# UoB-HPC/neutral

Measured on AMD Instinct MI355X. Metric: particle-steps/sec, higher is better.
Workload: dtype f64

## Files before the change

### neutral_amd/csrc/neutral_tiled.hip

```cpp
#include <cstdlib>
#include <cstring>
#include <type_traits>

#include "neutral_kernels.h"

#include "neutral_device.h"
#include "neutral_history.h"
#include "neutral_wave.h"

namespace neutral {

#ifndef NEUTRAL_STREAM_BLOCK
#define NEUTRAL_STREAM_BLOCK 1024
#endif
constexpr int kStreamBlock = NEUTRAL_STREAM_BLOCK;
constexpr int kChunkParticlesMax = 32768;
constexpr int kChunkParticlesMin = 1024;
constexpr int kStreamRefillMin = 56;
constexpr int kStreamRepeat = 64;
constexpr int kStreamRepeatOnePass = 128;
#ifdef NEUTRAL_NO_CARRIED_START
constexpr bool kCarriedStart = false;
#else
constexpr bool kCarriedStart = true;
// ... 342 lines not shown
                                                                    const unsigned* slot_of_id,
                                                                    ParticleView p, int n,
                                                                    const int* abort_flag,
                                                                    const unsigned* first_inactive,
                                                                    unsigned final_from,
                                                                    const unsigned* skip_ids,
                                                                    int partial_ok) {
  if (abort_flag && *abort_flag) {
    return;
  }
  for (long long kk = (long long)blockIdx.x * kSortBlock + threadIdx.x; kk < n; kk += (long long)gridDim.x * kSortBlock) {
    const int k = (int)kk;
    if (skip_ids && ((skip_ids[k >> 5] >> (k & 31)) & 1u)) {
      continue;
    }
    const unsigned slot = slot_of_id[k];
    if (slot >= (first_inactive ? *first_inactive : final_from)) {
      continue;
    }
    const rec_quad* const q = (const rec_quad*)__builtin_assume_aligned(&rec[slot], 16);
    ParticleRec r;
    rec_quad* const rq = (rec_quad*)&r;
    rq[0] = q[0];
    rq[1] = q[1];
    rq[2] = q[2];
    __builtin_nontemporal_store(r.x, &p.x[k]);
    __builtin_nontemporal_store(r.y, &p.y[k]);
    __builtin_nontemporal_store(r.dt_to_census, &p.dt_to_census[k]);
    __builtin_nontemporal_store(r.mfp_to_collision, &p.mfp_to_collision[k]);
    __builtin_nontemporal_store(r.cellx, &p.cellx[k]);
    __builtin_nontemporal_store(r.celly, &p.celly[k]);
    if (!partial_ok || (r.dead & kRecChanged)) {
      rq[3] = q[3];
      rq[4] = q[4];
      __builtin_nontemporal_store(r.omega_x, &p.omega_x[k]);
      __builtin_nontemporal_store(r.omega_y, &p.omega_y[k]);
      __builtin_nontemporal_store(r.energy, &p.energy[k]);
      __builtin_nontemporal_store(r.weight, &p.weight[k]);
      __builtin_nontemporal_store((record_state(r.dead) == kRecDead) ? 1 : 0, &p.dead[k]);
    }
  }
}

__global__ __launch_bounds__(1024) void tile_chunks_kernel(TiledArgs t) {
  __shared__ unsigned s_chunks[1024];
  constexpr int kStagedOffsets = 8192;
  __shared__ unsigned s_offset[kStagedOffsets + 2];
  const int tid = threadIdx.x;
  const bool staged = t.nsort + 1 <= kStagedOffsets;
  if (staged) {
    for (int i = tid; i <= t.nsort + 1; i += 1024) {
      s_offset[i] = t.tile_offset[i];
    }
    __syncthreads();
  }
  const unsigned* offset = staged ? s_offset : t.tile_offset;
  const unsigned nactive = offset[t.nsort];
  const int classes = t.reach_classes;
  long long per = (t.ntiles + 1023) / 1024;
  if (nactive > 0) {
    const long long per_sparse =
        ((long long)t.chunk_particles * (long long)t.ntiles + nactive - 1) / (long long)nactive;
    per = (per_sparse > per) ? per_sparse : per;
    constexpr long long kSweepTilesMax = 32;
    const long long floor_per = (t.ntiles + 1023) / 1024;
    const long long cap = (floor_per > kSweepTilesMax) ? floor_per : kSweepTilesMax;
    per = (per > cap) ? cap : per;
  }
  per = (per > t.ntiles) ? t.ntiles : per;
  const long long lo_ll = (long long)tid * per;
  const int lo = (lo_ll < t.ntiles) ? (int)lo_ll : t.ntiles;
  const int hi = (lo_ll + per < t.ntiles) ? (int)(lo_ll + per) : t.ntiles;
  const unsigned cp = (unsigned)t.chunk_particles;

  unsigned nch = 0;
  unsigned chunk = 0;
  unsigned nwindowed = 0;
  for (int sweep = 0; sweep < 2; ++sweep) {
    unsigned run_begin = 0, run_end = 0;
    auto emit = [&](unsigned begin, unsigned end, unsigned tile, unsigned windowed) {
      if (end <= begin) {
        return;
      }
      const unsigned parts = (end - begin + cp - 1) / cp;
      const unsigned size = (end - begin + parts - 1) / parts;
      for (unsigned b = begin; b < end; b += size) {
        const unsigned e = (b + size < end) ? b + size : end;
        if (sweep == 0) {
          nch++;
        } else {
          const unsigned w = (windowed && (e - b) >= (unsigned)t.window_min_particles) ? 1u : 0u;
          if (chunk < (unsigned)t.max_chunks) {
            t.chunks[chunk] = make_uint4(b, e, tile, w);
          }
          nwindowed += w;
          chunk++;
        }
      }
    };
    for (int i = lo; i < hi; ++i) {
      const unsigned begin = offset[i * classes];
      const unsigned end = offset[(i + 1) * classes];
      if (end - begin >= (unsigned)t.window_min_particles) {
        emit(run_begin, run_end, 0u, 0u);
        run_begin = run_end = end;
        emit(begin, end, (unsigned)i, 1u);
      } else {
        if (run_end == run_begin) {
          run_begin = begin;
        }
        run_end = end;
      }
    }
    emit(run_begin, run_end, 0u, 0u);
    if (sweep == 0) {
      s_chunks[tid] = nch;
      __syncthreads();
      for (int off = 1; off < 1024; off <<= 1) {
        const unsigned c0 = (tid >= off) ? s_chunks[tid - off] : 0;
        __syncthreads();
        s_chunks[tid] += c0;
        __syncthreads();
      }
      chunk = s_chunks[tid] - nch;
    }
  }
  if (nwindowed) {
    atomicAdd(&t.ctrl[kCtrlWindowed], nwindowed);
  }
  if (tid == 1023) {
    t.ctrl[kCtrlNumChunks] = s_chunks[1023];
    t.ctrl[kCtrlActive] = nactive;
    t.ctrl[kCtrlLive] = nactive;
    t.ctrl[kCtrlChunkHead] = 0;
    t.ctrl[kCtrlCollideCount] = 0;
    t.ctrl[kCtrlMigrants] = 0;
    if (t.pass == 0) {
      t.ctrl[kCtrlPassesUsed] = 1;
      t.ctrl[kCtrlEmigrants] = 0;
      t.ctrl[kCtrlFirstInactive] = offset[t.nsort];
    } else if (nactive > 0) {
      t.ctrl[kCtrlPassesUsed] = (unsigned)t.pass + 1u;
    }
  }
}

__global__ __launch_bounds__(kSortBlock) void tile_uniform_kernel(SolveArgs a, TiledArgs t, int window_cells) {
  __shared__ int s_differs;
  if (threadIdx.x == 0) {
    s_differs = 0;
  }
  __syncthreads();
  const int tile = (int)blockIdx.x;
  const int margin = (window_cells - (1 << t.tile_shift)) >> 1;
  int x0 = ((tile % t.tiles_x) << t.tile_shift) - margin - 1;
  int y0 = ((tile / t.tiles_x) << t.tile_shift) - margin - 1;
  int x1 = x0 + window_cells + 2;
  int y1 = y0 + window_cells + 2;
  x0 = (x0 < 0) ? 0 : x0;
  y0 = (y0 < 0) ? 0 : y0;
  x1 = (x1 > a.nx) ? a.nx : x1;
  y1 = (y1 > a.ny) ? a.ny : y1;
  const int w = x1 - x0;
  const int n = w * (y1 - y0);
  const long long first = __double_as_longlong(a.density[(size_t)y0 * a.nx + x0]);
  bool differs = false;
  for (int i = threadIdx.x; i < n; i += kSortBlock) {
    const int y = y0 + i / w;
    const int x = x0 + i % w;
    differs |= (__double_as_longlong(a.density[(size_t)y * a.nx + x]) != first);
  }
  if (__ballot(differs) != 0 && (threadIdx.x & 63) == 0) {
    s_differs = 1;
  }
  __syncthreads();
  if (threadIdx.x == 0) {
    t.tile_uniform[tile] = s_differs ? 0 : 1;
  }
}

__global__ __launch_bounds__(1024) void edges_check_kernel(SolveArgs a, TiledArgs t) {
  __shared__ int s_differs;
  if (threadIdx.x == 0) {
    s_differs = 0;
  }
  __syncthreads();
  bool differs = !(a.edge_dx > 0.0) || !(a.edge_dy > 0.0);
  for (int i = threadIdx.x; i <= a.nx; i += 1024) {
    differs |= __double_as_longlong(edge_from_formula(a.edge_dx, i + a.x_off)) !=
               __double_as_longlong(a.edgex[i + a.pad]);
  }
  for (int i = threadIdx.x; i <= a.ny; i += 1024) {
    differs |= __double_as_longlong(edge_from_formula(a.edge_dy, i + a.y_off)) !=
               __double_as_longlong(a.edgey[i + a.pad]);
  }
  if (__ballot(differs) != 0 && (threadIdx.x & 63) == 0) {
    s_differs = 1;
  }
  __syncthreads();
  if (threadIdx.x == 0) {
    *t.edges_computed = s_differs ? 0 : 1;
  }
}


__global__ __launch_bounds__(kSortBlock) void queue_reset_kernel(TiledArgs t) {
  const int tile = (int)blockIdx.x;
  unsigned used = t.queue_tail[tile];
  used = (used > t.queue_capacity) ? t.queue_capacity : used;
  unsigned* log = t.queue_entries + (size_t)tile * t.queue_capacity;
  for (unsigned i = threadIdx.x; i < used; i += kSortBlock) {
    log[i] = kQueueEmpty;
  }
  __syncthreads();
  if (threadIdx.x == 0) {
    t.queue_tail[tile] = 0u;
    t.queue_head[tile] = 0u;
  }
}

template <int kW>
__device__ __forceinline__ void flush_window(const SolveArgs& a, double* window, double* mesh,
                                             int ox, int oy) {
  constexpr int kS = kW + kWindowRowPad;
  for (int i = threadIdx.x; i < kW * kW; i += kStreamBlock) {
    const int at = (i / kW) * kS + (i % kW);
    const double v = window[at];
    window[at] = 0.0;
    if (v != 0.0) {
      const int gx = ox + (i % kW);
      const int gy = oy + (i / kW);
      if (gx >= 0 && gx < a.nx && gy >= 0 && gy < a.ny) {
        unsafeAtomicAdd(&mesh[gy * a.nx + gx], v);
      }
    }
  }
}

template <bool kSameTables, bool kWithIndex = true>
__host__ __device__ __forceinline__ size_t stream_lds_payload_bytes(const SolveArgs& a, int window_cells) {
  size_t lds = sizeof(double) * (size_t)window_cells;
  if (kWithIndex && a.scatter_index) {
    lds += sizeof(unsigned short) * (size_t)(a.scatter_index_n + 1);
  }
  if (kWithIndex && !kSameTables && a.absorb_index) {
    lds += sizeof(unsigned short) * (size_t)(a.absorb_index_n + 1);
  }
  return (lds + 15) & ~(size_t)15;
}
#ifdef NEUTRAL_PHASE_CLOCK
constexpr size_t kStreamLdsControlBytes = 64 + 16 * 9 * 8;
#else
constexpr size_t kStreamLdsControlBytes = 64;
#endif

__device__ __forceinline__ bool far_to_go(const History& h, const TiledArgs& t) {
  const double ahead = h.speed * h.dt_to_census;
  const double facets_ahead = ahead * (fabs(h.omega_x) * t.cells_per_x +
                                       fabs(h.omega_y) * t.cells_per_y);
  return facets_ahead > kMigrateMinFacets;
}

#ifdef NEUTRAL_PHASE_CLOCK
__device__ unsigned long long g_phase_clock[8];
#define PHASE_DECL                                                                              \
  unsigned long long* const lds_ph =                                                            \
      (unsigned long long*)((char*)lds_ctl + 64) + (threadIdx.x >> 6) * 9;                      \
  if ((threadIdx.x & 63) == 0) {                                                                \
    lds_ph[0] = __builtin_readcyclecounter();                                                   \
    for (int k = 1; k <= 8; ++k) lds_ph[k] = 0;                                                 \
  }
#define PHASE(k)                                                                                \
  do {                                                                                          \
    if ((int)(threadIdx.x & 63) == __builtin_ctzll(__builtin_amdgcn_ballot_w64(true))) {        \
      const unsigned long long ph_now = __builtin_readcyclecounter();                           \
      lds_ph[1 + (k)] += ph_now - lds_ph[0];                                                    \
      lds_ph[0] = ph_now;                                                                       \
    }                                                                                           \
  } while (0)
#define PHASE_REPORT                                                                            \
  if ((threadIdx.x & 63) == 0) {                                                                \
    for (int k = 0; k < 8; ++k) atomicAdd(&g_phase_clock[k], lds_ph[1 + k]);                    \
  }
extern "C" void neutral_hip_debug_phase_clock(unsigned long long* out8) {
  (void)hipDeviceSynchronize();
  (void)hipMemcpyFromSymbol(out8, HIP_SYMBOL(g_phase_clock), sizeof(unsigned long long) * 8);
  unsigned long long zero[8] = {0, 0, 0, 0, 0, 0, 0, 0};
  (void)hipMemcpyToSymbol(HIP_SYMBOL(g_phase_clock), zero, sizeof(zero));
}
#else
#define PHASE_DECL
#define PHASE(k)
#define PHASE_REPORT
#endif

static __device__ SpectrumParams d_spectrum = {};

static __global__ void spectrum_params_kernel(SpectrumParams p) { d_spectrum = p; }

static __device__ CurrentParams d_current = {nullptr, nullptr, nullptr};

static __global__ void current_params_kernel(CurrentParams p) { d_current = p; }

template <bool kSameTables, bool kFlux, bool kDomain, bool kChecked, bool kQueues, bool kSpectrum = false,
          bool kCurrent = false>
__global__ __launch_bounds__(kStreamBlock) void stream_kernel(SolveArgs a, TiledArgs t) {
  constexpr bool kCarried = kCarriedStart && kSameTables && !kDomain && !kQueues;
  constexpr int kW = WindowTallyT<kFlux, kCarried, false, kCurrent>::W;
  constexpr int kWindows = window_count(kFlux, kCurrent);
  extern __shared__ double lds_raw[];
  constexpr int kWindowDoubles = kW * (kW + kWindowRowPad);
  double* window = lds_raw;
  unsigned short* lds_index = (unsigned short*)(lds_raw + kWindows * kWindowDoubles);
  int* const lds_ctl = (int*)((char*)lds_raw + stream_lds_payload_bytes<kSameTables, !kCarried>(a, kWindows * kWindowDoubles));
  int& s_chunk = lds_ctl[0];
  int& s_end = lds_ctl[1];
  int& s_tile = lds_ctl[2];
  int& s_windowed = lds_ctl[3];
  int& s_cursor = lds_ctl[4];
  int& s_kind = lds_ctl[5];
  unsigned& s_best = ((unsigned*)lds_ctl)[6];
  int& s_best_tile = lds_ctl[7];

  if (a.abort_flag && *a.abort_flag) {
    return;
  }
  clock_stamp_begin(a.counters);
  CsLookup<const unsigned short*> ix{nullptr, nullptr};
  {
    int used = 0;
    if (!kCarried && a.scatter_index) {
      for (int i = threadIdx.x; i <= a.scatter_index_n; i += kStreamBlock) {
        lds_index[i] = a.scatter_index[i];
      }
      ix.scatter_index = lds_index;
      used = a.scatter_index_n + 1;
    }
    if (!kCarried && !kSameTables && a.absorb_index) {
      for (int i = threadIdx.x; i <= a.absorb_index_n; i += kStreamBlock) {
        lds_index[used + i] = a.absorb_index[i];
      }
      ix.absorb_index = lds_index + used;
    }
    for (int i = threadIdx.x; i < kWindows * kWindowDoubles; i += kStreamBlock) {
      window[i] = 0.0;
    }
  }
  WindowTallyT<kFlux, kCarried, kSpectrum, kCurrent> tally{(lds_double*)window, 0, 0, SpectrumView{},
                                                           kCurrent ? &d_current : nullptr};
  if (kSpectrum) {
    tally.spectrum = spectrum_view(&d_spectrum, (lds_double*)((char*)lds_ctl + kStreamLdsControlBytes));
    spectrum_bins_zero(tally.spectrum);
  }

  const int nchunks = (int)t.ctrl[kCtrlNumChunks];
  const bool edges_computed =
      t.edges_computed && __builtin_amdgcn_readfirstlane(*t.edges_computed) != 0;
  const bool budget_on = t.allow_migrate && (kQueues || t.ctrl[kCtrlWindowed] != 0);
  int cur_tile = -1;
  int win_ox = 0;
  int win_oy = 0;

  unsigned nfacets = 0;
  unsigned w_processed = 0;
  unsigned w_census = 0;
  unsigned w_migrants = 0;
  unsigned w_emigrants = 0;

  History h;
  h.ev = kEvEnd;
  spectrum_lane_start(h, tally);
  int pid = -1;

  const bool queues = kQueues && t.allow_migrate;
  const unsigned qcap = t.queue_capacity;
  unsigned w_ended = 0;
  unsigned w_hops = 0;
  unsigned w_overflows = 0;
  unsigned wg_batches = 0;
  unsigned wg_idle_polls = 0;
  enum : int { kWorkChunk = 0, kWorkQueue = 1, kWorkNone = 2 };

  PHASE_DECL
  for (;;) {
    if (queues && (threadIdx.x & 63) == 0 && w_ended) {
      atomicSub(&t.ctrl[kCtrlLive], w_ended);
    }
    w_ended = 0;
    unsigned polls = 0;
    for (;;) {
      __syncthreads();
      auto claim = [&](int tile, unsigned at_least) -> bool {
        for (;;) {
          const unsigned head = __hip_atomic_load(&t.queue_head[tile], __ATOMIC_RELAXED, __HIP_MEMORY_SCOPE_AGENT);
          unsigned tail = __hip_atomic_load(&t.queue_tail[tile], __ATOMIC_RELAXED, __HIP_MEMORY_SCOPE_AGENT);
          tail = (tail > qcap) ? qcap : tail;
          if (tail <= head || tail - head < at_least) {
            return false;
          }
          unsigned m = tail - head;
          m = (m > kQueueBatchMax) ? kQueueBatchMax : m;
          if (atomicCAS(&t.queue_head[tile], head, head + m) == head) {
            s_cursor = (int)head;
            s_end = (int)(head + m);
            s_tile = tile;
            s_windowed = 1;
            return true;
          }
        }
      };
      if (threadIdx.x == 0) {
        s_best = 0u;
        s_best_tile = -1;
        int kind = kWorkNone;
        if (queues && cur_tile >= 0 && claim(cur_tile, kQueueStayMin)) {
          kind = kWorkQueue;
          wg_batches++;
        }
        if (kind == kWorkNone &&
            __hip_atomic_load(&t.ctrl[kCtrlChunkHead], __ATOMIC_RELAXED, __HIP_MEMORY_SCOPE_AGENT) < (unsigned)nchunks) {
          const int c = (int)atomicAdd(&t.ctrl[kCtrlChunkHead], 1u);
          if (c < nchunks) {
            const uint4 ch = t.chunks[c];
            s_cursor = (int)ch.x;
            s_end = (int)ch.y;
            s_tile = (int)ch.z;
            s_windowed = (int)ch.w;
            kind = kWorkChunk;
          }
        }
        s_kind = kind;
      }
      __syncthreads();
      if (__builtin_amdgcn_readfirstlane(s_kind) != kWorkNone) {
        break;
      }
      if (!queues) {
        break;
      }
      {
        const int start = (cur_tile >= 0) ? cur_tile : (int)((blockIdx.x * 2654435761u) % (unsigned)t.ntiles);
        unsigned mine = 0u;
        int mine_tile = -1;
        for (int tile = (int)threadIdx.x; tile < t.ntiles; tile += kStreamBlock) {
          unsigned tail = __hip_atomic_load(&t.queue_tail[tile], __ATOMIC_RELAXED, __HIP_MEMORY_SCOPE_AGENT);
          const unsigned head = __hip_atomic_load(&t.queue_head[tile], __ATOMIC_RELAXED, __HIP_MEMORY_SCOPE_AGENT);
          tail = (tail > qcap) ? qcap : tail;
          if (tail > head) {
            const unsigned waiting = tail - head;
            unsigned key;
            if (waiting >= kQueueBatchMin) {
              int ahead = tile - start;
              ahead += (ahead < 0) ? t.ntiles : 0;
              key = 0x80000000u | (unsigned)(t.ntiles - ahead);
            } else {
              const unsigned salt = ((unsigned)tile * 2654435761u + blockIdx.x * 40503u + polls * 9973u) >> 22;
              key = (waiting << 10) | salt;
            }
            if (key > mine) {
              mine = key;
              mine_tile = tile;
            }
          }
        }
        unsigned most = mine;
#pragma unroll
        for (int off = 32; off > 0; off >>= 1) {
          const unsigned other = __shfl_xor(most, off, 64);
          most = (other > most) ? other : most;
        }
        const unsigned long long m_top = __ballot(most != 0u && mine == most);
        if (m_top != 0ull && __builtin_ctzll(m_top) == (int)(threadIdx.x & 63)) {
          atomicMax(&s_best, most);
        }
        __syncthreads();
        if (mine != 0u && mine == s_best) {
          s_best_tile = mine_tile;
        }
        __syncthreads();
      }
      if (threadIdx.x == 0) {
        int kind = kWorkNone;
        if (s_best != 0u && claim(s_best_tile, 1u)) {
          kind = kWorkQueue;
        }
        s_kind = kind;
        if (kind == kWorkQueue) {
          wg_batches++;
        }
        s_chunk = 0;
        if (kind == kWorkNone) {
          const unsigned live = __hip_atomic_load(&t.ctrl[kCtrlLive], __ATOMIC_RELAXED, __HIP_MEMORY_SCOPE_AGENT);
          if (live == 0u) {
            s_chunk = -1;
          } else if (s_best != 0u) {
          } else if (polls >= kQueueIdlePollsMax) {
            atomicAdd(&a.counters->aborted, 1u);
            s_chunk = -1;
          } else {
            wg_idle_polls++;
            const unsigned nap = (polls < 5u) ? polls : 5u;
            for (unsigned k = 0; k < (1u << nap); ++k) {
              __builtin_amdgcn_s_sleep(64);
            }
          }
        }
      }
      __syncthreads();
      if (__builtin_amdgcn_readfirstlane(s_kind) != kWorkNone || __builtin_amdgcn_readfirstlane(s_chunk) < 0) {
        break;
      }
      polls++;
    }
    const int work = __builtin_amdgcn_readfirstlane(s_kind);
    PHASE(0);
    if (work == kWorkNone) {
      break;
    }
    const bool from_queue = (work == kWorkQueue);
    const bool fresh = !from_queue && t.pass == 0;
    const int chunk_end = __builtin_amdgcn_readfirstlane(s_end);
    const int chunk_tile = __builtin_amdgcn_readfirstlane(s_tile);
    const bool windowed = (__builtin_amdgcn_readfirstlane(s_windowed) != 0);
    if (windowed && chunk_tile != cur_tile) {
      if (cur_tile >= 0) {
        flush_window<kW>(a, window, a.tally, win_ox, win_oy);
        if (kFlux) {
          flush_window<kW>(a, window + kWindowDoubles, a.flux_tally, win_ox, win_oy);
        }
        if (kCurrent) {
          flush_window<kW>(a, window + 2 * kWindowDoubles, d_current.jx, win_ox, win_oy);
          flush_window<kW>(a, window + 3 * kWindowDoubles, d_current.jy, win_ox, win_oy);
        }
      }
      cur_tile = chunk_tile;
      const int margin = (kW - (1 << t.tile_shift)) >> 1;
      win_ox = ((cur_tile % t.tiles_x) << t.tile_shift) - margin;
      win_oy = ((cur_tile / t.tiles_x) << t.tile_shift) - margin;
      __syncthreads();
    }
    PHASE(1);
    const bool uniform_window =
        windowed && t.tile_uniform &&
        __builtin_amdgcn_readfirstlane((int)t.tile_uniform[cur_tile]) != 0;
    double window_density = 0.0;
    if (kCarried && uniform_window) {
      const int tile_x = (cur_tile % t.tiles_x) << t.tile_shift;
      const int tile_y = (cur_tile / t.tiles_x) << t.tile_shift;
      window_density = a.density[(size_t)tile_y * (size_t)a.nx + (size_t)tile_x];
    }
    unsigned long long may_migrate =
        __builtin_amdgcn_readfirstlane((windowed && t.allow_migrate) ? 1 : 0) ? ~0ull : 0ull;
    asm volatile("" : "+s"(may_migrate));
    tally.ox = __builtin_amdgcn_readfirstlane(windowed ? win_ox : (1 << 30));
    tally.oy = __builtin_amdgcn_readfirstlane(windowed ? win_oy : (1 << 30));

    bool has = false;
    bool drained = false;
    for (;;) {
      const unsigned long long m_empty = __ballot(!has);
      const int n_empty = drained ? 0 : __popcll(m_empty);
      const int n_stream = 64 - __popcll(m_empty);
      if (n_empty + n_stream == 0) {
        break;
      }
      int park = kRecIdle;
      bool did_census = false;
      bool ended = false;
      if (n_empty >= t.refill_min || n_stream == 0) {
        int base = 0;
        if ((threadIdx.x & 63) == 0) {
          base = atomicAdd(&s_cursor, n_empty);
        }
        base = __builtin_amdgcn_readfirstlane(base);
        if (base >= chunk_end) {
          drained = true;
        } else {
          const int mine = base + lane_rank(m_empty);
          if (fresh) {
            const int left = chunk_end - base;
            w_processed += (unsigned)((n_empty < left) ? n_empty : left);
          }
          if (!has && mine < chunk_end) {
            unsigned src;
            if (from_queue) {
              const unsigned* place = t.queue_entries + ((size_t)chunk_tile * qcap + (size_t)mine);
              unsigned spins = 0;
              do {
                src = __hip_atomic_load(place, __ATOMIC_RELAXED, __HIP_MEMORY_SCOPE_AGENT);
              } while (src == kQueueEmpty && ++spins < (1u << 22));
            } else {
              src = t.order[mine];
            }
            if (src >= (unsigned)a.nparticles) {
              atomicAdd(&a.counters->aborted, 1u);
              ended = true;
            } else {
            pid = fresh ? mine : (int)src;
            double micro = 0.0, minus_log_rn0 = 0.0;
            if (kCarried) {
              const CarriedStart cs = fresh ? t.carried_in[src] : t.carried_out[src];
              micro = cs.micro;
              minus_log_rn0 = cs.minus_log_rn0;
            }
            bool bad_load = false;
            if (from_queue || (queues && !fresh)) {
              load_record_through(h, a, t.rec_out[src], true);
              if (from_queue) {
                const int want_tile = ((h.celly - a.y_off) >> t.tile_shift) * t.tiles_x + ((h.cellx - a.x_off) >> t.tile_shift);
                bad_load = (want_tile != chunk_tile) | (!kDomain && (h.id & ~kIdChanged) >= (unsigned)a.nparticles);
              }
            } else {
              load_record(h, a, fresh ? t.rec_in[src] : t.rec_out[src], !fresh);
            }
            if (fresh) {
              t.id_out[pid] = h.id;
              if (!kDomain && t.slots_by_id) {
                t.slot_of_id[h.id] = (unsigned)pid;
              }
              if (kCarried) {
                t.carried_out[pid].micro = micro;
              }
            }
            if (bad_load) {
              atomicAdd(&a.counters->aborted, 1u);
              ended = true;
            } else {
            if (kCarried) {
              if (fresh) {
                prologue_carried<kChecked>(h, a, micro, minus_log_rn0, uniform_window, window_density);
              } else {
                resume_carried<kChecked>(h, a, micro, uniform_window, window_density);
              }
            } else if (fresh) {
              prologue<kSameTables, kChecked>(h, a, ix);
            } else {
              resume<kSameTables, kChecked>(h, a, ix);
            }
            if (!kDomain) {
              h.counter = 1;
            }
            h.plain_div = 0;
            refresh_speed_reciprocal<kChecked>(h);
            refresh_mfp_reciprocal<kChecked>(h);
            h.dep_rate = deposit_rate(h, a);
            spectrum_regroup(h, tally);
            if (edges_computed) {
              load_targets<true>(h, a);
            } else {
              load_targets<false>(h, a);
            }
            decide_carried(h);
            h.nevents++;
            has = true;
            if (h.ev == kEvCollision) {
              park = kRecCollide;
            }
            }
            }
          }
        }
        PHASE(2);
      } else if (has) {
        if (h.ev == kEvFacet) {
          int crossed = 0;
          h.m_x_facet = __builtin_amdgcn_ballot_w64(h.x_facet != 0);

          auto run_facets = [&](auto uniform_density, auto computed_edges) {
          constexpr bool kUniform = decltype(uniform_density)::value;
          constexpr bool kEdges = decltype(computed_edges)::value;
          WindowCellTallyT<kFlux, kUniform, kCarried, kSpectrum, kCurrent> cell_tally{
              tally.window, (unsigned)(h.cellx - a.x_off - tally.ox),
              (unsigned)(h.celly - a.y_off - tally.oy), 0ull, tally.spectrum, tally.current_meshes};
          bool out_of_window = cell_tally.outside();
          cell_tally.m_outside = __builtin_amdgcn_ballot_w64(out_of_window);
          bool run = true;
          if ((cell_tally.m_outside & may_migrate) != 0) {
            asm volatile("");
            if (out_of_window) {
              run = !far_to_go(h, t);
            }
          }
          PHASE(3);
          if (run) {
#pragma unroll 1
            do {
              cross_facet<kChecked, true, kDomain ? 1 : 0, true, kEdges>(h, a, cell_tally);
              asm("v_add_u32_e32 %0, 1, %0" : "+v"(crossed));
              if (kDomain) {
                if (outside_domain(h, a)) {
                  park = kRecEmigrate;
                  break;
                }
              }
              cell_tally.lx = (unsigned)(h.cellx - a.x_off - tally.ox);
              cell_tally.ly = (unsigned)(h.celly - a.y_off - tally.oy);
              out_of_window = cell_tally.outside();
              cell_tally.m_outside = __builtin_amdgcn_ballot_w64(out_of_window);
              run = surely_next_is_facet(h) & (crossed < t.stream_repeat);
              if ((cell_tally.m_outside & may_migrate) != 0) {
                asm volatile("");
                if (out_of_window) {
                  run = run & !far_to_go(h, t);
                }
              }
            } while (run);
          }
          PHASE(5);
          };
          if (uniform_window) {
            if (edges_computed) {
              run_facets(std::true_type{}, std::true_type{});
            } else {
              run_facets(std::true_type{}, std::false_type{});
            }
          } else {
            if (edges_computed) {
              run_facets(std::false_type{}, std::true_type{});
            } else {
              run_facets(std::false_type{}, std::false_type{});
            }
          }
          decide_carried(h);
          park = (park == kRecIdle && h.ev == kEvCollision) ? (int)kRecCollide : park;
          if (windowed && t.allow_migrate && park == kRecIdle && h.ev == kEvFacet) {
            const unsigned lx = (unsigned)(h.cellx - a.x_off - tally.ox);
            const unsigned ly = (unsigned)(h.celly - a.y_off - tally.oy);
            if (!((lx < (unsigned)kW) & (ly < (unsigned)kW)) && far_to_go(h, t)) {
              park = kRecMigrate;
            }
          }
          nfacets += (unsigned)crossed;
          h.nevents += (unsigned)crossed;
          if (!windowed && budget_on && park == kRecIdle && h.ev == kEvFacet &&
              h.nevents >= kUnwindowedBudget) {
            const double ahead = h.speed * h.dt_to_census;
            if (ahead * (fabs(h.omega_x) * t.cells_per_x + fabs(h.omega_y) * t.cells_per_y) >
                kMigrateMinFacets) {
              park = kRecMigrate;
            }
          }
          if (h.nevents > kMaxEventsPerHistory && h.ev == kEvFacet && park == kRecIdle) {
            atomicAdd(&a.counters->aborted, 1u);
            h.ev = kEvEnd;
          }
          PHASE(3);
        } else {
          if (h.ev == kEvCensus) {
            census_streamed<kChecked>(h, a, tally);
          }
          store_record(h, a, t.rec_out[pid], kRecIdle);
          t.info_out[pid] = slot_summary(
              kRecIdle, h.cellx - a.x_off, h.celly - a.y_off, t.tiles_x, t.tile_shift,
              t.reach_classes > 1 ? reach_class(h.omega_x, h.omega_y, h.cellx - a.x_off,
                                                h.celly - a.y_off, t.tile_shift, kW, t.cells_per_x,
                                                t.cells_per_y)
                                  : 0u);
          has = false;
          ended = true;
          did_census = (h.ev == kEvCensus);
          PHASE(6);
        }
      }
      bool queued = false;
      const bool hop = queues && park == kRecMigrate;
      const unsigned long long m_hop = __ballot(hop);
      if (m_hop != 0ull) {
        int dest = 0;
        if (hop) {
          dest = ((h.celly - a.y_off) >> t.tile_shift) * t.tiles_x + ((h.cellx - a.x_off) >> t.tile_shift);
          if ((unsigned)dest >= (unsigned)t.ntiles || (unsigned)pid >= (unsigned)a.nparticles) {
            atomicAdd(&a.counters->aborted, 1u);
            dest = 0;
          }
          store_record_through(h, a, t.rec_out[(unsigned)pid < (unsigned)a.nparticles ? pid : 0], kRecMigrate);
        }
        int leader = -1;
        unsigned rank = 0, group = 0;
        unsigned long long todo = m_hop;
        while (todo != 0ull) {
          const int l = __builtin_ctzll(todo);
          const int tile_l = __builtin_amdgcn_readlane(dest, l);
          const unsigned long long same = __ballot(hop && dest == tile_l);
          if (hop && dest == tile_l) {
            leader = l;
            rank = (unsigned)lane_rank(same);
            group = (unsigned)__popcll(same);
          }
          todo &= ~same;
        }
        drain_stores();
        unsigned base = 0;
        if (hop && leader == (int)(threadIdx.x & 63)) {
          base = atomicAdd(&t.queue_tail[dest], group);
        }
        base = (unsigned)__shfl((int)base, leader < 0 ? 0 : leader, 64);
        if (hop) {
          const unsigned place = base + rank;
          if (place < qcap) {
            __hip_atomic_store(t.queue_entries + ((size_t)dest * qcap + (size_t)place), (unsigned)pid,
                               __ATOMIC_RELAXED, __HIP_MEMORY_SCOPE_AGENT);
            queued = true;
            has = false;
          }
        }
        w_hops += (unsigned)__popcll(__ballot(queued));
        w_overflows += (unsigned)__popcll(__ballot(hop && !queued));
      }
      if (park != kRecIdle && !queued) {
        if (!hop) {
          store_record(h, a, t.rec_out[pid], park);
        }
        t.info_out[pid] = slot_summary(
            park, h.cellx - a.x_off, h.celly - a.y_off, t.tiles_x, t.tile_shift,
            (t.reach_classes > 1 && park == kRecMigrate)
                ? reach_class(h.omega_x, h.omega_y, h.cellx - a.x_off, h.celly - a.y_off,
                              t.tile_shift, kW, t.cells_per_x, t.cells_per_y)
                : 0u);
        has = false;
        ended = true;
      }
      PHASE(7);
      w_ended += (unsigned)__popcll(__ballot(ended));
      w_migrants += (unsigned)__popcll(__ballot(park == kRecMigrate && !queued));
      if (kDomain) {
        w_emigrants += (unsigned)__popcll(__ballot(park == kRecEmigrate));
      }
      w_census += (unsigned)__popcll(__ballot(did_census));
    }
  }
  PHASE(0);
  PHASE_REPORT
  if ((threadIdx.x & 63) == 0 && w_migrants) {
    atomicAdd(&t.ctrl[kCtrlMigrants], w_migrants);
  }
  if ((threadIdx.x & 63) == 0 && w_hops) {
    atomicAdd(&t.ctrl[kCtrlHops], w_hops);
  }
  if ((threadIdx.x & 63) == 0 && w_overflows) {
    atomicAdd(&t.ctrl[kCtrlOverflows], w_overflows);
  }
  if (threadIdx.x == 0 && wg_batches) {
    atomicAdd(&t.ctrl[kCtrlBatches], wg_batches);
  }
  if (threadIdx.x == 0 && wg_idle_polls) {
    atomicAdd(&t.ctrl[kCtrlIdlePolls], wg_idle_polls);
  }
  if (kDomain && (threadIdx.x & 63) == 0 && w_emigrants) {
    atomicAdd(&t.ctrl[kCtrlEmigrants], w_emigrants);
  }
  if (cur_tile >= 0) {
    flush_window<kW>(a, window, a.tally, win_ox, win_oy);
    if (kFlux) {
      flush_window<kW>(a, window + kWindowDoubles, a.flux_tally, win_ox, win_oy);
    }
    if (kCurrent) {
      flush_window<kW>(a, window + 2 * kWindowDoubles, d_current.jx, win_ox, win_oy);
      flush_window<kW>(a, window + 3 * kWindowDoubles, d_current.jy, win_ox, win_oy);
    }
  }
  spectrum_finish(h, tally, d_spectrum.buffer, a.inv_ntotal_particles);
  {
    const unsigned wf = wave_sum_u32(nfacets);
    if ((threadIdx.x & 63) == 0) {
      if (w_processed) atomicAdd(&a.counters->nprocessed, (unsigned long long)w_processed);
      if (wf) atomicAdd(&a.counters->nfacets, (unsigned long long)wf);
      if (w_census) atomicAdd(&a.counters->ncensus, (unsigned long long)w_census);
    }
  }
  clock_stamp_end(a.counters);
}


__device__ __forceinline__ int owner_rank(const DomainGrid& d, int cellx, int celly) {
  int rx = cellx / d.bx;
  int ry = celly / d.by;
  rx = (rx < 0) ? 0 : ((rx >= d.px) ? d.px - 1 : rx);
  ry = (ry < 0) ? 0 : ((ry >= d.py) ? d.py - 1 : ry);
  return ry * d.px + rx;
}

__global__ __launch_bounds__(kSortBlock) void emigrant_count_kernel(const ParticleRec* rec,
                                                                    const unsigned* info, int n,
                                                                    DomainGrid d, unsigned* counts) {
  const int i = blockIdx.x * kSortBlock + threadIdx.x;
  if (i < n && summary_state(info[i]) == kRecEmigrate) {
    atomicAdd(&counts[owner_rank(d, rec[i].cellx, rec[i].celly)], 1u);
  }
}

__global__ __launch_bounds__(kSortBlock) void emigrant_pack_kernel(ParticleRec* rec, unsigned* info,
                                                                   int n, DomainGrid d,
                                                                   const unsigned* offset,
                                                                   unsigned* cursor,
                                                                   ParticleRec* send, int tiles_x,
                                                                   int tile_shift,
                                                                   unsigned* free_slots,
                                                                   unsigned* nfree) {
  const int i = blockIdx.x * kSortBlock + threadIdx.x;
  if (i < n && summary_state(info[i]) == kRecEmigrate) {
    ParticleRec r = rec[i];
    const int dest = owner_rank(d, r.cellx, r.celly);
    const unsigned k = atomicAdd(&cursor[dest], 1u);
    free_slots[atomicAdd(nfree, 1u)] = (unsigned)i;
    const unsigned counter = record_counter(r.dead);
    r.dead = record_word(kRecMigrate, counter);
    send[offset[dest] + k] = r;
    rec[i].dead = record_word(kRecGone, 0u);
    info[i] = slot_summary(kRecGone, 0, 0, tiles_x, tile_shift);
  }
}

__global__ __launch_bounds__(kSortBlock) void immigrant_append_kernel(const ParticleRec* recv,
                                                                      int nrecv, ParticleRec* rec,
                                                                      unsigned* info, unsigned* ids,
                                                                      int first_slot, int x_off,
                                                                      int y_off, int tiles_x,
                                                                      int tile_shift,
                                                                      unsigned* migrants,
                                                                      const unsigned* free_slots,
                                                                      int nfree, int reuse) {
  const int j = blockIdx.x * kSortBlock + threadIdx.x;
  if (j == 0) {
    atomicAdd(migrants, (unsigned)nrecv);
  }
  if (j < nrecv) {
    const ParticleRec r = recv[j];
    const int slot = (j < reuse) ? (int)free_slots[nfree - 1 - j] : first_slot + (j - reuse);
    rec[slot] = r;
    ids[slot] = r.id;
    info[slot] = slot_summary(kRecMigrate, r.cellx - x_off, r.celly - y_off, tiles_x, tile_shift);
  }
}

__global__ __launch_bounds__(kSortBlock) void compact_records_kernel(
    const ParticleRec* rec, const unsigned* info, const unsigned* ids, int n, ParticleRec* rec_to,
    unsigned* info_to, unsigned* ids_to, unsigned* cursor) {
  const int i = blockIdx.x * kSortBlock + threadIdx.x;
  const bool keep = i < n && summary_state(info[i]) != kRecGone;
  const unsigned long long m = __ballot(keep);
  unsigned base = 0;
  if ((threadIdx.x & 63) == 0 && m) {
    base = atomicAdd(cursor, (unsigned)__popcll(m));
  }
  base = __builtin_amdgcn_readfirstlane(base);
  if (keep) {
    const unsigned j = base + (unsigned)lane_rank(m);
    rec_to[j] = rec[i];
    info_to[j] = info[i];
    ids_to[j] = ids[i];
  }
}

__global__ __launch_bounds__(kSortBlock) void import_by_slot_kernel(ParticleView p,
                                                                    const unsigned* keys,
                                                                    ParticleRec* rec, unsigned* info,
                                                                    unsigned* ids, int tiles_x,
                                                                    int tile_shift, int x_off,
                                                                    int y_off, int n) {
  const int i = blockIdx.x * kSortBlock + threadIdx.x;
  if (i < n) {
    ParticleRec r;
    r.x = p.x[i];
    r.y = p.y[i];
    r.omega_x = p.omega_x[i];
    r.omega_y = p.omega_y[i];
    r.energy = p.energy[i];
    r.weight = p.weight[i];
    r.dt_to_census = p.dt_to_census[i];
    r.mfp_to_collision = p.mfp_to_collision[i];
    r.cellx = p.cellx[i];
    r.celly = p.celly[i];
    r.id = keys[i];
    r.dead = p.dead[i] ? kRecDead : kRecIdle;
    rec[i] = r;
    ids[i] = r.id;
    info[i] = slot_summary(p.dead[i] ? kRecDead : kRecIdle, r.cellx - x_off, r.celly - y_off,
                           tiles_x, tile_shift);
  }
}

__global__ __launch_bounds__(kSortBlock) void export_by_slot_kernel(const ParticleRec* rec,
                                                                    ParticleView p, unsigned* keys,
                                                                    int n) {
  const int k = blockIdx.x * kSortBlock + threadIdx.x;
  if (k < n) {
    const ParticleRec r = rec[k];
    p.x[k] = r.x;
    p.y[k] = r.y;
    p.omega_x[k] = r.omega_x;
    p.omega_y[k] = r.omega_y;
    p.energy[k] = r.energy;
    p.weight[k] = r.weight;
    p.dt_to_census[k] = r.dt_to_census;
    p.mfp_to_collision[k] = r.mfp_to_collision;
    p.cellx[k] = r.cellx;
    p.celly[k] = r.celly;
    p.dead[k] = (record_state(r.dead) == kRecDead) ? 1 : 0;
    keys[k] = r.id;
  }
}

hipError_t launch_emigrant_count(const TiledArgs& t, int n, const DomainGrid& d, unsigned* counts,
                                 hipStream_t stream) {
  if (n > 0) {
    hipLaunchKernelGGL(emigrant_count_kernel, dim3((n + kSortBlock - 1) / kSortBlock),
                       dim3(kSortBlock), 0, stream, t.rec_out, t.info_out, n, d, counts);
  }
  return hipGetLastError();
}

hipError_t launch_emigrant_pack(const TiledArgs& t, int n, const DomainGrid& d,
                                const unsigned* offset, unsigned* cursor, ParticleRec* send,
                                unsigned* free_slots, unsigned* nfree, hipStream_t stream) {
  if (n > 0) {
    hipLaunchKernelGGL(emigrant_pack_kernel, dim3((n + kSortBlock - 1) / kSortBlock),
                       dim3(kSortBlock), 0, stream, t.rec_out, t.info_out, n, d, offset, cursor,
                       send, t.tiles_x, t.tile_shift, free_slots, nfree);
    (void)hipMemsetAsync(&t.ctrl[kCtrlEmigrants], 0, sizeof(unsigned), stream);
  }
  return hipGetLastError();
}

hipError_t launch_immigrant_append(const TiledArgs& t, const ParticleRec* recv, int nrecv,
                                   int first_slot, int x_off, int y_off,
                                   const unsigned* free_slots, int nfree, int reuse,
                                   hipStream_t stream) {
  if (nrecv > 0) {
    hipLaunchKernelGGL(immigrant_append_kernel, dim3((nrecv + kSortBlock - 1) / kSortBlock),
                       dim3(kSortBlock), 0, stream, recv, nrecv, t.rec_out, t.info_out, t.id_out,
                       first_slot, x_off, y_off, t.tiles_x, t.tile_shift, &t.ctrl[kCtrlMigrants],
                       free_slots, nfree, reuse);
  }
  return hipGetLastError();
}

hipError_t launch_compact_records(const TiledArgs& t, int n, unsigned* cursor, hipStream_t stream) {
  (void)hipMemsetAsync(cursor, 0, sizeof(unsigned), stream);
  if (n > 0) {
    hipLaunchKernelGGL(compact_records_kernel, dim3((n + kSortBlock - 1) / kSortBlock),
                       dim3(kSortBlock), 0, stream, t.rec_out, t.info_out, t.id_out, n, t.rec_in,
                       t.info_in, t.id_in, cursor);
  }
  return hipGetLastError();
}

hipError_t launch_import_by_slot(const ParticleView& p, const unsigned* keys, const TiledArgs& t,
                                 int x_off, int y_off, int n, hipStream_t stream) {
  if (n > 0) {
    hipLaunchKernelGGL(import_by_slot_kernel, dim3((n + kSortBlock - 1) / kSortBlock),
                       dim3(kSortBlock), 0, stream, p, keys, t.rec_in, t.info_in, t.id_in, t.tiles_x,
                       t.tile_shift, x_off, y_off, n);
  }
  return hipGetLastError();
}

hipError_t launch_export_by_slot(const ParticleRec* rec, const ParticleView& p, unsigned* keys,
                                 int n, hipStream_t stream) {
  if (n > 0) {
    hipLaunchKernelGGL(export_by_slot_kernel, dim3((n + kSortBlock - 1) / kSortBlock),
                       dim3(kSortBlock), 0, stream, rec, p, keys, n);
  }
  return hipGetLastError();
}


static bool stream_stages_no_index(const SolveArgs& a, const TiledArgs& t) {
  return kCarriedStart && a.same_tables && !a.decomposed && !t.queue_entries;
}

static bool current_on = false;

hipError_t use_current_tiled(const CurrentParams* p, hipStream_t stream) {
  current_on = p != nullptr;
  if (p) {
    hipLaunchKernelGGL(current_params_kernel, dim3(1), dim3(1), 0, stream, *p);
  }
  return hipGetLastError();
}

static int stream_window_cells(const SolveArgs& a, const TiledArgs& t) {
  return window_cells(a.flux_tally != nullptr, stream_stages_no_index(a, t), current_on);
}

static int spectrum_groups = 0;

hipError_t use_spectrum_tiled(const SpectrumParams* p, hipStream_t stream) {
  spectrum_groups = p ? p->ngroups : 0;
  if (p) {
    hipLaunchKernelGGL(spectrum_params_kernel, dim3(1), dim3(1), 0, stream, *p);
  }
  return hipGetLastError();
}

size_t tiled_lds_bytes(const SolveArgs& a, const TiledArgs& t) {
  const int w = stream_window_cells(a, t);
  const int cells = window_count(a.flux_tally != nullptr, current_on) * w * (w + kWindowRowPad);
  const bool carried = stream_stages_no_index(a, t);
  return (carried ? stream_lds_payload_bytes<true, false>(a, cells)
                  : a.same_tables ? stream_lds_payload_bytes<true>(a, cells)
                                  : stream_lds_payload_bytes<false>(a, cells)) +
         kStreamLdsControlBytes + sizeof(double) * 2 * (size_t)spectrum_groups;
}

int tiled_chunk_particles(int nparticles, int compute_units) {
  long long c = (long long)nparticles / ((long long)compute_units * 6);
  if (c > kChunkParticlesMax) c = kChunkParticlesMax;
  if (c < kChunkParticlesMin) c = kChunkParticlesMin;
  return (int)c;
}

int tiled_tile_shift(int nx, int ny, int nparticles, bool with_flux) {
  const int largest = with_flux ? 6 : 7;
  const char* force = getenv("NEUTRAL_TILE_CELLS");
  if (force) {
    const int cells = atoi(force);
    for (int shift = 4; shift <= largest; ++shift) {
      if (cells == (1 << shift)) {
        return shift;
      }
    }
  }
  const double density = (double)nparticles / ((double)nx * (double)ny);
  const int shift = (density >= 8.0) ? 4 : (density >= 2.0) ? 5 : (density >= 0.5) ? 6 : 7;
  return shift < largest ? shift : largest;
}

int tiled_window_min_particles(int tile_shift) {
  const char* force = getenv("NEUTRAL_WINDOW_MIN_PARTICLES");
  if (force) {
    return atoi(force);
  }
  return (tile_shift >= 7) ? 64 : (2048 >> (tile_shift - 4));
}

void tiled_geometry(int nx, int ny, int nparticles, int tile_shift, int* tiles_x, int* tiles_y,
                    int* max_chunks) {
  const int tile = 1 << tile_shift;
  *tiles_x = (nx + tile - 1) / tile;
  *tiles_y = (ny + tile - 1) / tile;
  *max_chunks = (*tiles_x) * (*tiles_y) + nparticles / kChunkParticlesMin + 1;
}

hipError_t launch_import_records(const ParticleView& p, ParticleRec* rec, unsigned* info,
                                 unsigned* slot_of_id, unsigned* ids, int tiles_x, int tile_shift,
                                 int x_off, int y_off, int n, hipStream_t stream) {
  if (n > 0) {
    hipLaunchKernelGGL(import_records_kernel, dim3((n + kSortBlock - 1) / kSortBlock),
                       dim3(kSortBlock), 0, stream, p, rec, info, slot_of_id, ids, tiles_x, tile_shift,
                       x_off, y_off, n);
  }
  return hipGetLastError();
}

hipError_t launch_refresh_micro(const SolveArgs& a, const TiledArgs& t, hipStream_t stream) {
  if (t.sort_end > 0) {
    hipLaunchKernelGGL(refresh_micro_kernel, dim3((t.sort_end + kSortBlock - 1) / kSortBlock),
                       dim3(kSortBlock), 0, stream, a, t);
  }
  return hipGetLastError();
}

bool tiled_uses_carried(const SolveArgs& a, const TiledArgs& t) {
  return kCarriedStart && a.same_tables && !a.decomposed && !t.queue_entries && t.carried_in &&
         t.carried_out;
}

hipError_t launch_export_records(const ParticleRec* rec, const unsigned* slot_of_id,
                                 const ParticleView& p, int n, hipStream_t stream,
                                 const int* abort_flag, const unsigned* first_inactive,
                                 unsigned final_from, const unsigned* skip_ids, int max_blocks,
                                 bool partial_ok) {
  if (n > 0) {
    int grid = (n + kSortBlock - 1) / kSortBlock;
    grid = (max_blocks > 0 && grid > max_blocks) ? max_blocks : grid;
    hipLaunchKernelGGL(export_records_kernel, dim3(grid), dim3(kSortBlock), 0, stream, rec,
                       slot_of_id, p, n, abort_flag, first_inactive, final_from, skip_ids, partial_ok ? 1 : 0);
  }
  return hipGetLastError();
}

const unsigned* tiled_first_inactive(const TiledArgs& t) { return &t.ctrl[kCtrlFirstInactive]; }

static hipError_t enqueue_stream_pass(const SolveArgs& a, TiledArgs& t, int pass, int cus,
                                      size_t lds, hipStream_t stream, hipEvent_t after_sort) {
  t.pass = pass;
  t.allow_migrate = (pass + 1 < kMaxStreamPasses) ? 1 : 0;
  const int grid_n = (a.nparticles + kSortBlock - 1) / kSortBlock;
  const int grid_seg = t.sort_end > 0 ? (t.sort_end + kSortSegment - 1) / kSortSegment : 1;
  const int nbins = t.nsort + 1;
  const size_t lds_bins = (nbins <= kSortLdsBins) ? sizeof(unsigned) * (size_t)nbins : 0;
  hipLaunchKernelGGL(tile_count_kernel, dim3(grid_seg), dim3(kSortBlock), lds_bins, stream, a, t);
  hipLaunchKernelGGL(tile_scan_kernel, dim3(1), dim3(1024), 0, stream, t);
  hipLaunchKernelGGL(tile_scatter_kernel, dim3(grid_seg), dim3(kSortBlock), 2 * lds_bins, stream, a,
                     t);
  hipLaunchKernelGGL(tile_chunks_kernel, dim3(1), dim3(1024), 0, stream, t);
  if (pass == 0) {
    hipLaunchKernelGGL(copy_inactive_kernel, dim3(grid_n < 8192 ? grid_n : 8192), dim3(kSortBlock), 0, stream,
                       a, t);
    if (after_sort) {
      (void)hipEventRecord(after_sort, stream);
    }
  }
  if (t.queue_entries) {
    hipLaunchKernelGGL(queue_reset_kernel, dim3(t.ntiles), dim3(kSortBlock), 0, stream, t);
  }
  auto launch = [&](auto kernel) {
    (void)hipFuncSetAttribute((const void*)kernel, hipFuncAttributeMaxDynamicSharedMemorySize,
                              (int)lds);
    hipLaunchKernelGGL(kernel, dim3(cus), dim3(kStreamBlock), lds, stream, a, t);
  };
  auto launch_for = [&](auto queues_tag, auto spectrum_tag, auto current_tag) {
    constexpr bool kQ = decltype(queues_tag)::value;
    constexpr bool kS = decltype(spectrum_tag)::value;
    constexpr bool kK = decltype(current_tag)::value;
    switch ((a.checked ? 8 : 0) | (a.same_tables ? 4 : 0) | (a.flux_tally ? 2 : 0) |
            (a.decomposed ? 1 : 0)) {
      case 15: launch(stream_kernel<true, true, true, true, kQ, kS, kK>); break;
      case 14: launch(stream_kernel<true, true, false, true, kQ, kS, kK>); break;
      case 13: launch(stream_kernel<true, false, true, true, kQ, kS>); break;
      case 12: launch(stream_kernel<true, false, false, true, kQ, kS>); break;
      case 11: launch(stream_kernel<false, true, true, true, kQ, kS, kK>); break;
      case 10: launch(stream_kernel<false, true, false, true, kQ, kS, kK>); break;
      case 9: launch(stream_kernel<false, false, true, true, kQ, kS>); break;
      case 8: launch(stream_kernel<false, false, false, true, kQ, kS>); break;
      case 7: launch(stream_kernel<true, true, true, false, kQ, kS, kK>); break;
      case 6: launch(stream_kernel<true, true, false, false, kQ, kS, kK>); break;
      case 5: launch(stream_kernel<true, false, true, false, kQ, kS>); break;
      case 4: launch(stream_kernel<true, false, false, false, kQ, kS>); break;
      case 3: launch(stream_kernel<false, true, true, false, kQ, kS, kK>); break;
      case 2: launch(stream_kernel<false, true, false, false, kQ, kS, kK>); break;
      case 1: launch(stream_kernel<false, false, true, false, kQ, kS>); break;
      default: launch(stream_kernel<false, false, false, false, kQ, kS>); break;
    }
  };
  auto launch_queues = [&](auto spectrum_tag, auto current_tag) {
    if (t.queue_entries) {
      launch_for(std::true_type{}, spectrum_tag, current_tag);
    } else {
      launch_for(std::false_type{}, spectrum_tag, current_tag);
    }
  };
  auto launch_spectrum = [&](auto current_tag) {
    if (spectrum_groups > 0) {
      launch_queues(std::true_type{}, current_tag);
    } else {
      launch_queues(std::false_type{}, current_tag);
    }
  };
  if (current_on && !a.flux_tally) {
    return hipErrorInvalidValue;
  }
  if (current_on) {
    launch_spectrum(std::true_type{});
  } else {
    launch_spectrum(std::false_type{});
  }
  return hipGetLastError();
}

hipError_t launch_solve_tiled(const SolveArgs& a, TiledArgs& t, hipStream_t stream,
                              const TiledPlan& plan, int first_pass, hipEvent_t after_sort,
                              hipEvent_t after_stream, hipEvent_t after_collect,
                              int* passes_enqueued, const SplitExport* split) {
  if (passes_enqueued) {
    *passes_enqueued = first_pass;
  }
  if (a.nparticles <= 0) {
    if (after_sort && first_pass == 0) (void)hipEventRecord(after_sort, stream);
    if (after_stream) (void)hipEventRecord(after_stream, stream);
    if (after_collect) (void)hipEventRecord(after_collect, stream);
    return hipSuccess;
  }
  if (a.decomposed || t.sort_end > a.nparticles || t.mirror_end < t.sort_end) {
    t.sort_end = a.nparticles;
    t.mirror_end = a.nparticles;
  }
  const int cus = a.compute_units > 0 ? a.compute_units : 256;
  t.chunk_particles = tiled_chunk_particles(a.nparticles, cus);
  t.refill_min = kStreamRefillMin;
  t.stream_repeat = (plan.stream_passes <= 2) ? kStreamRepeatOnePass : kStreamRepeat;
  t.carried = tiled_uses_carried(a, t) ? 1 : 0;
  const size_t lds = tiled_lds_bytes(a, t);
  (void)hipFuncSetAttribute((const void*)tile_scatter_kernel,
                            hipFuncAttributeMaxDynamicSharedMemorySize,
                            (int)(2 * sizeof(unsigned) * kSortLdsBins));

  if (first_pass == 0 && t.edges_computed) {
    hipLaunchKernelGGL(edges_check_kernel, dim3(1), dim3(1024), 0, stream, a, t);
  }
  if (first_pass == 0 && t.tile_uniform && a.pad == 0) {
    hipLaunchKernelGGL(tile_uniform_kernel, dim3(t.ntiles), dim3(kSortBlock), 0, stream, a, t,
                       stream_window_cells(a, t));
  } else if (first_pass == 0 && t.tile_uniform) {
    (void)hipMemsetAsync(t.tile_uniform, 0, (size_t)t.ntiles, stream);
  }
  int pass = first_pass;
  for (int k = 0; k < plan.stream_passes && pass < kMaxStreamPasses; ++k, ++pass) {
    const hipError_t err = enqueue_stream_pass(a, t, pass, cus, lds, stream, after_sort);
    if (err != hipSuccess) {
      return err;
    }
  }
  if (passes_enqueued) {
    *passes_enqueued = pass;
  }
  if (after_stream) {
    (void)hipEventRecord(after_stream, stream);
  }

  hipLaunchKernelGGL(collect_suspended_kernel,
                     dim3(t.sort_end > 0 ? (t.sort_end + kSortSegment - 1) / kSortSegment : 1),
                     dim3(kSortBlock), 0, stream, a, t, t.info_out);
  if (after_collect) {
    (void)hipEventRecord(after_collect, stream);
  }
  SolveArgs c = a;
  c.blocks_per_cu = plan.blocks_per_cu;
  c.counters = a.counters + 1;
  c.queue = t.collide_queue;
  c.queue_len = &t.ctrl[kCtrlCollideCount];
  c.rec = t.rec_out;
  c.slot_info = t.info_out;
  c.tiles_x = t.tiles_x;
  c.tile_shift = t.tile_shift;
  c.susp = t.susp;
  c.susp_track = t.susp_track;
  c.carried = t.carried ? t.carried_out : nullptr;
  c.steal = t.steal;
  c.emigrants = &t.ctrl[kCtrlEmigrants];
  if (t.fine_index && c.same_tables) {
    c.scatter_index = t.fine_index;
    c.scatter_index_n = t.fine_index_n;
    c.scatter_index_base = t.fine_index_base;
    c.index_shift = t.fine_index_shift;
  }
  return launch_solve(c, kVariantEventSorted, stream);
}

hipError_t launch_split_export(const SolveArgs& a, const TiledArgs& t, const SplitExport& split,
                               hipEvent_t after_collect) {
  (void)hipStreamWaitEvent(split.side, after_collect, 0);
  (void)launch_export_records(t.rec_out, t.slot_of_id, split.p, a.nparticles, split.side, a.abort_flag,
                              split.skip_long_dead ? &t.ctrl[kCtrlFirstInactive] : nullptr, 0xFFFFFFFFu,
                              t.susp_ids, 0, split.skip_long_dead != 0);
  (void)hipEventRecord(split.done, split.side);
  return hipGetLastError();
}


}
```

Baseline: 147.5 billion.

## Cut SGPR/VGPR pressure by reloading kernargs and moving wave counters to LDS

```diff
diff --git a/neutral_amd/csrc/neutral_tiled.hip b/neutral_amd/csrc/neutral_tiled.hip
--- a/neutral_amd/csrc/neutral_tiled.hip
+++ b/neutral_amd/csrc/neutral_tiled.hip
@@ -668,6 +668,13 @@
 
 static __global__ void current_params_kernel(CurrentParams p) { d_current = p; }
 
+typedef const __attribute__((address_space(4))) TiledArgs* TiledArgsAgain;
+__device__ __forceinline__ TiledArgsAgain tiled_args_again() {
+  unsigned long long p = (unsigned long long)__builtin_amdgcn_kernarg_segment_ptr();
+  asm volatile("" : "+s"(p));
+  return (TiledArgsAgain)(p + ((sizeof(SolveArgs) + 7) & ~(size_t)7));
+}
+
 template <bool kSameTables, bool kFlux, bool kDomain, bool kChecked, bool kQueues, bool kSpectrum = false,
           bool kCurrent = false>
 __global__ __launch_bounds__(kStreamBlock) void stream_kernel(SolveArgs a, TiledArgs t) {
@@ -678,7 +685,11 @@
   constexpr int kWindowDoubles = kW * (kW + kWindowRowPad);
   double* window = lds_raw;
   unsigned short* lds_index = (unsigned short*)(lds_raw + kWindows * kWindowDoubles);
-  int* const lds_ctl = (int*)((char*)lds_raw + stream_lds_payload_bytes<kSameTables, !kCarried>(a, kWindows * kWindowDoubles));
+  unsigned ctl_offset = (unsigned)stream_lds_payload_bytes<kSameTables, !kCarried>(a, kWindows * kWindowDoubles);
+  if (kSameTables || !kFlux) {
+    asm volatile("" : "+s"(ctl_offset));
+  }
+  int* const lds_ctl = (int*)((char*)lds_raw + ctl_offset);
   int& s_chunk = lds_ctl[0];
   int& s_end = lds_ctl[1];
   int& s_tile = lds_ctl[2];
@@ -687,6 +698,9 @@
   int& s_kind = lds_ctl[5];
   unsigned& s_best = ((unsigned*)lds_ctl)[6];
   int& s_best_tile = lds_ctl[7];
+  unsigned& s_processed = ((unsigned*)lds_ctl)[8];
+  unsigned& s_census = ((unsigned*)lds_ctl)[9];
+  unsigned& s_migrants = ((unsigned*)lds_ctl)[10];
 
   if (a.abort_flag && *a.abort_flag) {
     return;
@@ -728,9 +742,11 @@
   int win_oy = 0;
 
   unsigned nfacets = 0;
-  unsigned w_processed = 0;
-  unsigned w_census = 0;
-  unsigned w_migrants = 0;
+  if (threadIdx.x == 0) {
+    s_processed = 0u;
+    s_census = 0u;
+    s_migrants = 0u;
+  }
   unsigned w_emigrants = 0;
 
   History h;
@@ -883,8 +899,9 @@
     if (work == kWorkNone) {
       break;
     }
+    const TiledArgsAgain tc = tiled_args_again();
     const bool from_queue = (work == kWorkQueue);
-    const bool fresh = !from_queue && t.pass == 0;
+    const bool fresh = !from_queue && tc->pass == 0;
     const int chunk_end = __builtin_amdgcn_readfirstlane(s_end);
     const int chunk_tile = __builtin_amdgcn_readfirstlane(s_tile);
     const bool windowed = (__builtin_amdgcn_readfirstlane(s_windowed) != 0);
@@ -900,19 +917,19 @@
         }
       }
       cur_tile = chunk_tile;
-      const int margin = (kW - (1 << t.tile_shift)) >> 1;
-      win_ox = ((cur_tile % t.tiles_x) << t.tile_shift) - margin;
-      win_oy = ((cur_tile / t.tiles_x) << t.tile_shift) - margin;
+      const int margin = (kW - (1 << tc->tile_shift)) >> 1;
+      win_ox = ((cur_tile % tc->tiles_x) << tc->tile_shift) - margin;
+      win_oy = ((cur_tile / tc->tiles_x) << tc->tile_shift) - margin;
       __syncthreads();
     }
     PHASE(1);
     const bool uniform_window =
-        windowed && t.tile_uniform &&
-        __builtin_amdgcn_readfirstlane((int)t.tile_uniform[cur_tile]) != 0;
+        windowed && tc->tile_uniform &&
+        __builtin_amdgcn_readfirstlane((int)tc->tile_uniform[cur_tile]) != 0;
     double window_density = 0.0;
     if (kCarried && uniform_window) {
-      const int tile_x = (cur_tile % t.tiles_x) << t.tile_shift;
-      const int tile_y = (cur_tile / t.tiles_x) << t.tile_shift;
+      const int tile_x = (cur_tile % tc->tiles_x) << tc->tile_shift;
+      const int tile_y = (cur_tile / tc->tiles_x) << tc->tile_shift;
       window_density = a.density[(size_t)tile_y * (size_t)a.nx + (size_t)tile_x];
     }
     unsigned long long may_migrate =
@@ -934,6 +951,7 @@
       bool did_census = false;
       bool ended = false;
       if (n_empty >= t.refill_min || n_stream == 0) {
+        const TiledArgsAgain tr = tiled_args_again();
         int base = 0;
         if ((threadIdx.x & 63) == 0) {
           base = atomicAdd(&s_cursor, n_empty);
@@ -943,9 +961,9 @@
           drained = true;
         } else {
           const int mine = base + lane_rank(m_empty);
-          if (fresh) {
+          if (fresh && (threadIdx.x & 63) == 0) {
             const int left = chunk_end - base;
-            w_processed += (unsigned)((n_empty < left) ? n_empty : left);
+            atomicAdd(&s_processed, (unsigned)((n_empty < left) ? n_empty : left));
           }
           if (!has && mine < chunk_end) {
             unsigned src;
@@ -956,7 +974,7 @@
                 src = __hip_atomic_load(place, __ATOMIC_RELAXED, __HIP_MEMORY_SCOPE_AGENT);
               } while (src == kQueueEmpty && ++spins < (1u << 22));
             } else {
-              src = t.order[mine];
+              src = tr->order[mine];
             }
             if (src >= (unsigned)a.nparticles) {
               atomicAdd(&a.counters->aborted, 1u);
@@ -965,27 +983,27 @@
             pid = fresh ? mine : (int)src;
             double micro = 0.0, minus_log_rn0 = 0.0;
             if (kCarried) {
-              const CarriedStart cs = fresh ? t.carried_in[src] : t.carried_out[src];
+              const CarriedStart cs = fresh ? tr->carried_in[src] : tr->carried_out[src];
               micro = cs.micro;
               minus_log_rn0 = cs.minus_log_rn0;
             }
             bool bad_load = false;
             if (from_queue || (queues && !fresh)) {
-              load_record_through(h, a, t.rec_out[src], true);
+              load_record_through(h, a, tr->rec_out[src], true);
               if (from_queue) {
                 const int want_tile = ((h.celly - a.y_off) >> t.tile_shift) * t.tiles_x + ((h.cellx - a.x_off) >> t.tile_shift);
                 bad_load = (want_tile != chunk_tile) | (!kDomain && (h.id & ~kIdChanged) >= (unsigned)a.nparticles);
               }
             } else {
-              load_record(h, a, fresh ? t.rec_in[src] : t.rec_out[src], !fresh);
+              load_record(h, a, fresh ? tr->rec_in[src] : tr->rec_out[src], !fresh);
             }
             if (fresh) {
-              t.id_out[pid] = h.id;
-              if (!kDomain && t.slots_by_id) {
-                t.slot_of_id[h.id] = (unsigned)pid;
+              tr->id_out[pid] = h.id;
+              if (!kDomain && tr->slots_by_id) {
+                tr->slot_of_id[h.id] = (unsigned)pid;
               }
               if (kCarried) {
-                t.carried_out[pid].micro = micro;
+                tr->carried_out[pid].micro = micro;
               }
             }
             if (bad_load) {
@@ -1112,13 +1130,14 @@
           }
           PHASE(3);
         } else {
+          const TiledArgsAgain tr = tiled_args_again();
           if (h.ev == kEvCensus) {
             census_streamed<kChecked>(h, a, tally);
           }
-          store_record(h, a, t.rec_out[pid], kRecIdle);
-          t.info_out[pid] = slot_summary(
+          store_record(h, a, tr->rec_out[pid], kRecIdle);
+          tr->info_out[pid] = slot_summary(
               kRecIdle, h.cellx - a.x_off, h.celly - a.y_off, t.tiles_x, t.tile_shift,
-              t.reach_classes > 1 ? reach_class(h.omega_x, h.omega_y, h.cellx - a.x_off,
+              tr->reach_classes > 1 ? reach_class(h.omega_x, h.omega_y, h.cellx - a.x_off,
                                                 h.celly - a.y_off, t.tile_shift, kW, t.cells_per_x,
                                                 t.cells_per_y)
                                   : 0u);
@@ -1174,12 +1193,13 @@
         w_overflows += (unsigned)__popcll(__ballot(hop && !queued));
       }
       if (park != kRecIdle && !queued) {
+        const TiledArgsAgain tr = tiled_args_again();
         if (!hop) {
-          store_record(h, a, t.rec_out[pid], park);
-        }
-        t.info_out[pid] = slot_summary(
+          store_record(h, a, tr->rec_out[pid], park);
+        }
+        tr->info_out[pid] = slot_summary(
             park, h.cellx - a.x_off, h.celly - a.y_off, t.tiles_x, t.tile_shift,
-            (t.reach_classes > 1 && park == kRecMigrate)
+            (tr->reach_classes > 1 && park == kRecMigrate)
                 ? reach_class(h.omega_x, h.omega_y, h.cellx - a.x_off, h.celly - a.y_off,
                               t.tile_shift, kW, t.cells_per_x, t.cells_per_y)
                 : 0u);
@@ -1188,17 +1208,24 @@
       }
       PHASE(7);
       w_ended += (unsigned)__popcll(__ballot(ended));
-      w_migrants += (unsigned)__popcll(__ballot(park == kRecMigrate && !queued));
+      {
+        const unsigned long long m_migrants = __ballot(park == kRecMigrate && !queued);
+        const unsigned long long m_census = __ballot(did_census);
+        if ((m_migrants | m_census) != 0ull && (threadIdx.x & 63) == 0) {
+          if (m_migrants != 0ull) atomicAdd(&s_migrants, (unsigned)__popcll(m_migrants));
+          if (m_census != 0ull) atomicAdd(&s_census, (unsigned)__popcll(m_census));
+        }
+      }
       if (kDomain) {
         w_emigrants += (unsigned)__popcll(__ballot(park == kRecEmigrate));
       }
-      w_census += (unsigned)__popcll(__ballot(did_census));
     }
   }
   PHASE(0);
   PHASE_REPORT
-  if ((threadIdx.x & 63) == 0 && w_migrants) {
-    atomicAdd(&t.ctrl[kCtrlMigrants], w_migrants);
+  __syncthreads();
+  if (threadIdx.x == 0 && s_migrants) {
+    atomicAdd(&t.ctrl[kCtrlMigrants], s_migrants);
   }
   if ((threadIdx.x & 63) == 0 && w_hops) {
     atomicAdd(&t.ctrl[kCtrlHops], w_hops);
@@ -1229,9 +1256,11 @@
   {
     const unsigned wf = wave_sum_u32(nfacets);
     if ((threadIdx.x & 63) == 0) {
-      if (w_processed) atomicAdd(&a.counters->nprocessed, (unsigned long long)w_processed);
       if (wf) atomicAdd(&a.counters->nfacets, (unsigned long long)wf);
-      if (w_census) atomicAdd(&a.counters->ncensus, (unsigned long long)w_census);
+    }
+    if (threadIdx.x == 0) {
+      if (s_processed) atomicAdd(&a.counters->nprocessed, (unsigned long long)s_processed);
+      if (s_census) atomicAdd(&a.counters->ncensus, (unsigned long long)s_census);
     }
   }
   clock_stamp_end(a.counters);
@@ -1550,6 +1579,9 @@
 
 static hipError_t enqueue_stream_pass(const SolveArgs& a, TiledArgs& t, int pass, int cus,
                                       size_t lds, hipStream_t stream, hipEvent_t after_sort) {
+  if (stream_stages_no_index(a, t) != (t.carried != 0)) {
+    return hipErrorInvalidValue;
+  }
   t.pass = pass;
   t.allow_migrate = (pass + 1 < kMaxStreamPasses) ? 1 : 0;
   const int grid_n = (a.nparticles + kSortBlock - 1) / kSortBlock;
```

New measurement: 146.7 billion. No clear change (-0.5%).
